# danpovey/quantization

Measured on AMD Instinct MI355X. Metric: vectors encoded/sec at dim=512, 8 codebooks; uint8 codes bit-exact vs ref, higher is better.
Workload: dtype f32 (products: exact 30-bit fixed point on the i8 MFMA); 1 GPU; Quantizer.encode, dim=512, bytes_per_frame=8, codebook_size=256, refine_indexes_iters=5, batch=65536 fp32 Gaussian vectors per GPU (BASELINE.json configs[1]), seeded synthetic codebooks; global_batch=65536, parallelism=batch-sharded x1, no collective

## Files before the change

quantization_amd/csrc/mcq_api.hip:

```cpp
#include "../../include/mcq.h"
#include "../../include/mcq_residual.h"
#include "../../include/mcq_probe.h"
#include "../../include/mcq_wide.h"
#include "../../include/mcq_rerank.h"
#include "mcq_kernels.h"
#include "mcq_fix_kernels.h"
#include "mcq_loss_kernels.h"
#include "mcq_tf_kernels.h"
#include "mcq_pass16_kernels.h"
#include "mcq_train_kernels.h"
#include "mcq_search_kernels.h"
#include "mcq_range_kernels.h"
#include "mcq_wide_kernels.h"
#include "mcq_rerank_kernels.h"

#include <cstdlib>
#include <iterator>
#include <type_traits>
#include <utility>
#include <vector>

using namespace mcq;

namespace {
// ... 179 lines not shown
    void untimed() { open = -1; }
    void end(int category) {
        if (only >= 0 && category != only) { open = -1; return; }
        hipEvent_t e;
        (void)hipEventCreate(&e);
        (void)hipEventRecord(e, stream);
        ev.push_back(e);
        first.push_back(open);
        last.push_back((int)ev.size() - 1);
        cat.push_back(category);
        open = (int)ev.size() - 1;
    }
};

thread_local int g_last_launches = 0;

#define MCQ_LAUNCH_CHECK()                               \
    do {                                                 \
        hipError_t e_ = hipGetLastError();               \
        if (e_ != hipSuccess) return (int)e_;            \
        ++g_last_launches;                               \
    } while (0)

inline int launch_rc() {
    const hipError_t e = hipGetLastError();
    return e == hipSuccess ? 0 : (int)e;
}
inline int counted_launch_rc() { MCQ_LAUNCH_CHECK(); return 0; }

template <typename F>
int launch_in_pieces(long B, int threads_per_row, F &&launch) {
    const long piece = (long)kPieceRows * 64 / (threads_per_row > 64 ? threads_per_row : 64);
    for (long at = 0; at < B; at += piece)
        if (const int rc = launch(at, B - at < piece ? B - at : piece)) return rc;
    return 0;
}

template <int... Vs, typename F>
int pick(int v, F &&f) {
    int rc = MCQ_EUNSUPPORTED;
    (void)((v == Vs && ((rc = f(std::integral_constant<int, Vs>{})), true)) || ...);
    return rc;
}
template <typename F>
int pick_bool(bool b, F &&f) { return b ? f(std::true_type{}) : f(std::false_type{}); }

struct Pair { int a, b; };
template <const auto &Table, typename F, size_t... I>
int pick_pair(int a, int b, F &&f, std::index_sequence<I...>) {
    int rc = MCQ_EUNSUPPORTED;
    (void)((a == Table[I].a && b == Table[I].b &&
            ((rc = f(std::integral_constant<int, Table[I].a>{}, std::integral_constant<int, Table[I].b>{})), true)) || ...);
    return rc;
}
template <const auto &Table, typename F>
int pick_pair(int a, int b, F &&f) { return pick_pair<Table>(a, b, f, std::make_index_sequence<std::size(Table)>{}); }
template <size_t R>
bool in_pairs(const Pair (&table)[R], int a, int b) {
    for (const Pair &p : table) if (p.a == a && p.b == b) return true;
    return false;
}

int allow_dynamic_lds(bool (&allowed)[64], const void *kernel, int bytes) {
    int dev = 0;
    if (hipGetDevice(&dev) != hipSuccess || dev < 0 || dev >= 64) dev = 63;
    if (!allowed[dev] || dev == 63) {
        const hipError_t attr = hipFuncSetAttribute(kernel, hipFuncAttributeMaxDynamicSharedMemorySize, bytes);
        if (attr != hipSuccess) return (int)attr;
        allowed[dev] = true;
    }
    return 0;
}

struct Timed {
    Prof *const prof;
    const int cat;
    Timed(Prof *p, int c) : prof(p), cat(c) { if (prof) prof->begin(cat); }
    ~Timed() { if (prof) prof->end(cat); }
    Timed(const Timed &) = delete;
};

FixRowsArgs fix_rows_args(const float *src, int xh, long R, int D, long ld, int8_t *planes, int *exps, float *xx,
                          const float *bias_src = nullptr, float *bias_dst = nullptr, const float *sub = nullptr,
                          long sub_per = 0, long sub_ld = 0, const float *dot_vec = nullptr, float *dot_out = nullptr) {
    return FixRowsArgs{src, xh, R, fix_round_rows(R), D, ld, fix_round_cols(D), planes, exps, xx, bias_src, bias_dst,
                       sub, sub_per, sub_ld, dot_vec, dot_out, nullptr};
}

int launch_fix_rows(const float *src, int xh, long R, int D, long ld, int8_t *planes, int *exps, float *xx, hipStream_t st,
                    const float *sub = nullptr, unsigned *clear = nullptr) {
    FixRowsArgs a = fix_rows_args(src, xh, R, D, ld, planes, exps, xx, nullptr, nullptr, sub, 0, 0);
    a.clear = clear;
    hipLaunchKernelGGL(k_fix_rows<4>, dim3((unsigned)(a.Rp / 4)), dim3(256), 0, st, a);
    return counted_launch_rc();
}

int launch_fix_rows2(const FixRowsArgs &a, const FixRowsArgs &b, hipStream_t st) {
    const unsigned na = (unsigned)(a.Rp / 4), nb = (unsigned)(b.Rp / 4);
    hipLaunchKernelGGL(k_fix_rows2<4>, dim3(na + nb), dim3(256), 0, st, a, b, na);
    return counted_launch_rc();
}

template <int MODE>
int launch_fgemm(FixGemm g, hipStream_t st) {
    static bool allowed[64] = {};
    constexpr int lds = MODE == FG_SCREEN ? kFixLdsScreen : kFixLds;
    if (const int rc = allow_dynamic_lds(allowed, reinterpret_cast<const void *>(&k_fgemm<MODE>), lds)) return rc;
    const long MT = g.RA / kFixTile, NT = g.RB / kFixTile;
    const int H = (MODE != FG_STORE && g.K > kFixTile) ? g.K / kFixTile : 1;
    const long big = g.walk_rows ? NT : MT, small_units = (g.walk_rows ? MT : NT) / H;
    long units = (big + 7) / 8 * small_units;
    if (units > 32) units = 32;
    hipLaunchKernelGGL((k_fgemm<MODE>), dim3((unsigned)(8 * units)), dim3(512), lds, st, g);
    return counted_launch_rc();
}

int launch_xc(const int8_t *xf, const int *xe, long B, const int8_t *Cf, const int *Ce, long nk, int D, float *out,
              hipStream_t st) {
    FixGemm g{};
    g.A = xf; g.ea = xe; g.RA = fix_round_rows(B); g.M = B;
    g.B = Cf; g.eb = Ce; g.RB = fix_round_rows(nk); g.N = nk;
    g.Dq = fix_round_cols(D);
    g.walk_rows = 0;
    g.out = out; g.ldo = nk;
    return launch_fgemm<FG_STORE>(g, st);
}

inline bool exact_logits_forced() {
    static const bool on = getenv("MCQ_EXACT_LOGITS") && atoi(getenv("MCQ_EXACT_LOGITS")) != 0;
    return on;
}

int launch_logits(const int8_t *xf, const int *xe, long B, const Prepared &P, int N, int K, int D, float lscale,
                  const float *lscale_ptr, float *logits, void *idx, hipStream_t st, unsigned *und_cnt = nullptr,
                  unsigned *und_list = nullptr) {
    const long nk = (long)N * K;
    FixGemm g{};
    g.A = P.Wf; g.ea = P.We; g.RA = fix_round_rows(nk); g.M = nk;
    g.B = xf; g.eb = xe; g.RB = fix_round_rows(B); g.N = B;
    g.Dq = fix_round_cols(D);
    g.walk_rows = 1;
    g.bias = P.bias; g.wmu = P.wmu; g.lscale = lscale; g.lscale_ptr = lscale_ptr;
    g.logits = logits; g.ldo = nk; g.idx = idx; g.idx_wide = K > 256 ? 1 : 0; g.K = K; g.ncb = N;
    if (und_cnt == nullptr) return launch_fgemm<FG_LOGITS>(g, st);
    if (logits != nullptr) return MCQ_EINVAL;
    g.und_cnt = und_cnt; g.und_list = und_list; g.und_cap = (unsigned)(B * N);
    const int rc = launch_fgemm<FG_SCREEN>(g, st);
    if (rc) return rc;
    FixRecheck r{};
    r.W = P.Wf; r.X = xf; r.ew = P.We; r.ex = xe; r.RW = g.RA; r.RX = g.RB; r.Dq = g.Dq;
    r.bias = P.bias; r.wmu = P.wmu; r.lscale_ptr = lscale_ptr; r.lscale = lscale;
    r.idx = idx; r.idx_wide = g.idx_wide; r.K = K; r.ncb = N; r.cnt = und_cnt; r.list = und_list; r.cap = g.und_cap;
    const long waves = B * N;
    hipLaunchKernelGGL(k_fscreen_recheck, dim3((unsigned)(waves < 4096 ? (waves + 3) / 4 : 1024)), dim3(256), 0, st, r);
    return counted_launch_rc();
}

constexpr unsigned kCapStage0 = 32768, kCapWave = 65536;
inline unsigned pass_grid(unsigned full, bool capped, unsigned cap) { return (capped && full > cap) ? cap : full; }

template <typename CT>
int launch_tf_stage0(int K, int N, const float *G, const float *XC, const CT *idx, const float *R, const float *Q, long B, int keep,
                     CT *ent, float *S, CT *fin, const int *nact, const int *map, hipStream_t st, bool capped) {
    const unsigned vgrid = (unsigned)(((B + 3) / 4) * N);
    const dim3 grid(pass_grid(vgrid, capped, kCapStage0)), block(256);
    auto with_k = [&](auto kk) {
        constexpr int KK = kk;
        return pick<1, 2, 4, 8, 16, 32, 64>(N, [&](auto nn) {
            constexpr int NN = nn;
            if constexpr ((KK == 16 && NN >= 4) || KK * NN > kMaxRows) return MCQ_EUNSUPPORTED;
            else return pick_bool(capped, [&](auto strided) {
                constexpr bool STRIDED = strided;
                hipLaunchKernelGGL((k_tf_stage0<KK, NN, STRIDED>), grid, block, 0, st, G, XC, idx, R, Q, B, keep, ent, S, fin, nact, map, vgrid);
                return counted_launch_rc();
            });
        });
    };
    if constexpr (sizeof(CT) == 1) {
        if (K == 16 && N >= 4) {
            const dim3 grid16((unsigned)((B * (N / 4) + 3) / 4));
            return pick<4, 8, 16, 32, 64>(N, [&](auto nn) {
                constexpr int NN = nn;
                hipLaunchKernelGGL((k_tf_stage0_k16<NN>), grid16, block, 0, st, G, XC, idx, R, Q, B, keep, ent, S, nact, map);
                return counted_launch_rc();
            });
        }
        return pick<16, 32, 64, 128, 256>(K, with_k);
    } else {
        return pick<512, 1024>(K, with_k);
    }
}

template <typename CT>
int launch_tf_er(int N, const float *G, const float *XC, const CT *idx, const float *xx, long B, int K, float *E, float *R,
                 float *gterms, long stride, const int *nact, const int *map, hipStream_t st, int form = -1) {
    const dim3 grid((unsigned)((B + 3) / 4)), block(256);
    const bool direct = form < 0 ? B <= 8192 : form == 0;
    return pick<1, 2, 4, 8, 16, 32, 64>(N, [&](auto nn) {
        constexpr int NN = nn, VG = 4 * (64 / NN);
        if constexpr (sizeof(CT) == 2 && NN * 512 > kMaxRows) return MCQ_EUNSUPPORTED;
        else {
            constexpr bool DENSE = sizeof(CT) == 1 && (NN == 4 || NN == 8 || NN == 16);
            if (!direct) {
                const long per = DENSE ? 256 : VG;
                hipLaunchKernelGGL((k_tf_gram_terms<NN, CT, DENSE>), dim3((unsigned)(((B + per - 1) / per) * NN)), block, 0, st, G, idx, B, K,
                                   gterms, nact, stride);
                if (const int rc = counted_launch_rc()) return rc;
                if constexpr (DENSE) {
                    hipLaunchKernelGGL((k_tf_er<NN, CT, true>), dim3((unsigned)((B + VG - 1) / VG)), block, 0, st, gterms, XC, idx, xx, B, K,
                                       E, R, nact, map, static_cast<const float *>(nullptr), stride);
                    return counted_launch_rc();
                }
            }
            hipLaunchKernelGGL((k_tf_er<NN, CT>), grid, block, 0, st, gterms, XC, idx, xx, B, K, E, R, nact, map,
                               direct ? G : static_cast<const float *>(nullptr), stride);
            return counted_launch_rc();
        }
    });
}

constexpr Pair kTfUpLists[] = {{16, 32}, {32, 32}, {32, 64}, {8, 16}, {16, 16}};
constexpr Pair kTfCombLists[] = {{16, 32}, {32, 32}, {32, 64}, {64, 64}, {8, 16}, {16, 16}};

template <typename CT>
constexpr bool tf_comb_reached(int kh, int kc, bool last) {
    const bool wide = sizeof(CT) == 2;
    if (kh == 8 || kc == 16) return !wide && !(kh == kc && last);
    if (kh == 64) return !wide;
    if (kh == kc) return !(last && wide);
    return !(kc == 64 && wide && !last);
}

int launch_tf_up(int kh, int kc, const TfLists &L, long B, int N, int u, int ntab, int per, const float *in, float *out,
                 const int *nact, hipStream_t st) {
    return pick_pair<kTfUpLists>(kh, kc, [&](auto a, auto c) {
        constexpr int KH = a, KC = c;
        hipLaunchKernelGGL((k_tf_up<KH, KC>), dim3((unsigned)(B * ntab)), dim3(64), 0, st, L, B, N, u, ntab, per, in, out, nact);
        return counted_launch_rc();
    });
}

template <typename CT>
int launch_tf_comb(int kh, int kc, const float *E, const TfLists &L, long B, int N, int v, int keep, const float *tabs,
                   CT *fin, const int *nact, hipStream_t st, bool capped) {
    if (fin == nullptr) capped = false;
    const dim3 grid(pass_grid((unsigned)(B * (N >> (v + 1))), capped, kCapWave)), block(64);
    return pick_pair<kTfCombLists>(kh, kc, [&](auto a, auto c) {
        return pick_bool(fin != nullptr, [&](auto last) {
            constexpr int KH = decltype(a)::value, KC = decltype(c)::value;
            constexpr bool LAST = last;
            if constexpr (!tf_comb_reached<CT>(KH, KC, LAST)) return MCQ_EUNSUPPORTED;
            else return pick_bool(capped, [&](auto strided) {
                constexpr bool STRIDED = strided;
                if constexpr (STRIDED && !LAST) return MCQ_EUNSUPPORTED;
                else {
                    hipLaunchKernelGGL((k_tf_comb<KH, KC, LAST, CT, STRIDED>), grid, block, 0, st, E, L, B, N, v, keep, tabs, fin, nact);
                    return counted_launch_rc();
                }
            });
        });
    });
}

enum { CAT_LOGITS = 0, CAT_XX = 1, CAT_STAGE0 = 2, CAT_XC = 3, CAT_LEVEL0 = 4, CAT_LEVEL1 = 5, CAT_TABLES = 6, CAT_COMBINE = 7,
       CAT_TABLES_UP = 8, CAT_COMBINE_UP = 9, CAT_ER = 10, CAT_LEVEL1_FUSED = 11, CAT_TAIL = 12, CAT_COUNT = 13 };
const char *const kCatNames[CAT_COUNT] = {
    "logits_product_argmax",
    "frames_to_limbs",
    "stage0_tables",
    "xc_product",
    "combine_level0",
    "combine_level1",
    "tables_level1",
    "combine_level2",
    "tables_upper_levels",
    "combine_upper_levels",
    "residual_energies",
    "level1_combines_and_tables",
    "encode_tail",
};

template <typename CT, typename F>
int pick_leaf_lists(int K, F &&f) {
    if constexpr (sizeof(CT) == 1) return pick<8, 16>(K == 16 ? 8 : 16, f);
    else return pick<16>(16, f);
}
inline bool pass16_enabled() {
    static const bool on = !(getenv("MCQ_PASS16") && atoi(getenv("MCQ_PASS16")) == 0);
    return on;
}
inline long skip_min_batch() {
    const char *v = getenv("MCQ_SKIP_MIN_BATCH");
    return v ? atol(v) : 8192;
}
constexpr long kErDenseMin = 16384;
inline long er_dense_min() {
    const char *v = getenv("MCQ_ER_DENSE_MIN");
    return v ? atol(v) : kErDenseMin;
}
constexpr long kLazyTablesMin = 16384;
inline long lazy_tables_min() {
    const char *v = getenv("MCQ_LAZY_TABLES_MIN");
    return v ? atol(v) : kLazyTablesMin;
}

template <typename CT>
int run_tf_combines(const float *G, const CT *idx_cur, CT *idx_new, const WorkspaceT<CT> &w, const TfLists &L, long B, int N,
// ... 1737 lines not shown
```

quantization_amd/csrc/mcq_fix_kernels.h:

```cpp
#pragma once
#include "mcq_kernels.h"

namespace mcq {

typedef int i32x4 __attribute__((ext_vector_type(4)));
typedef int i32x16 __attribute__((ext_vector_type(16)));

constexpr int kFixTile = 128;
constexpr int kFixColPad = 128;
constexpr int kFixRing = 4;
constexpr int kFixSlot = 32768;
constexpr int kFixOperand = 16384;
constexpr int kFixInfo = kFixRing * kFixSlot;
constexpr int kFixLds = kFixInfo + 4096;
constexpr int kFixLdsScreen = kFixLds + 1024;

__host__ __device__ inline long fix_round_rows(long r) { return (r + kFixTile - 1) / kFixTile * kFixTile; }
__host__ __device__ inline int fix_round_cols(int d) { return (d + kFixColPad - 1) / kFixColPad * kFixColPad; }
__host__ __device__ inline size_t fix_plane_bytes(long R, int D) { return (size_t)fix_round_rows(R) * fix_round_cols(D) * 4; }

__device__ __forceinline__ int fix_q(float v, int e) {
    float s = ldexpf(v, 30 - e);
    s = fminf(fmaxf(s, -1073741824.0f), 1073741824.0f);
    return (int)rintf(s);
}

struct FixRowsArgs {
    const float *src;
    int xh;
    long R, Rp;
    int D;
    long ld;
    int Dq;
    int8_t *planes;
    int *exps;
    float *xx;
    const float *bias_src;
    float *bias_dst;
    const float *sub;
    long sub_per, sub_ld;
    const float *dot_vec;
    float *dot_out;
    unsigned *clear;
};

template <int RW, bool DOT>
__device__ __forceinline__ void fix_rows_body(const FixRowsArgs &a, unsigned bid) {
    const float *__restrict__ src = a.src;
    const int xh = a.xh, D = a.D, Dq = a.Dq;
    const long R = a.R, Rp = a.Rp, ld = a.ld;
    float *__restrict__ xx = a.xx;
    const float *__restrict__ bias_src = a.bias_src;
    float *__restrict__ bias_dst = a.bias_dst;
    const float *__restrict__ sub = a.sub;
    int8_t *__restrict__ planes = a.planes;
    constexpr int RPW = RW / 4;
    __shared__ __attribute__((aligned(16))) unsigned tile[128 * RW * 4];
    __shared__ int es[RW];
    const int tid = threadIdx.x, lane = tid & 63, wave = tid >> 6;
    const long row0 = (long)bid * RW;
    if (bias_src && tid < RW && row0 + tid < R) bias_dst[row0 + tid] = bias_src[row0 + tid];
    if (a.clear && bid == 0 && tid == 0) *a.clear = 0u;
    const _Float16 *srch = reinterpret_cast<const _Float16 *>(src);
    const bool vec_ok = ((ld & 3) == 0) && ((D & 3) == 0) && ((reinterpret_cast<uintptr_t>(src) & (xh ? 7 : 15)) == 0);
    auto load4 = [&](long row, int q) -> f32x4 {
        f32x4 v = {0.f, 0.f, 0.f, 0.f};
        if (row >= R || 4 * q >= D) return v;
        if (vec_ok) return xh ? load_h4(srch + row * ld + 4 * q) : *reinterpret_cast<const f32x4 *>(src + row * ld + 4 * q);
#pragma unroll
        for (int c = 0; c < 4; ++c)
            if (4 * q + c < D) v[c] = xh ? (float)srch[row * ld + 4 * q + c] : src[row * ld + 4 * q + c];
        return v;
    };
    auto vec4 = [&](const float *p, int q) -> f32x4 {
        f32x4 v = {0.f, 0.f, 0.f, 0.f};
        if (4 * q >= D) return v;
        if (((D & 3) == 0) && ((reinterpret_cast<uintptr_t>(p) & 15) == 0)) return *reinterpret_cast<const f32x4 *>(p + 4 * q);
#pragma unroll
        for (int c = 0; c < 4; ++c)
            if (4 * q + c < D) v[c] = p[4 * q + c];
        return v;
    };
    auto sub4 = [&](long row, int q) -> f32x4 {
        if (!sub || row >= R) return f32x4{0.f, 0.f, 0.f, 0.f};
        return vec4(sub + (a.sub_per ? (row / a.sub_per) * a.sub_ld : 0), q);
    };
    int ev = 0;
    if (DOT && a.dot_vec) {
        float mv = 0.f;
        for (int q = lane; q < (D + 3) / 4; q += 64) {
            const f32x4 v = vec4(a.dot_vec, q);
#pragma unroll
            for (int c = 0; c < 4; ++c) mv = fmaxf(mv, fabsf(v[c]));
        }
        for (int s = 32; s >= 1; s >>= 1) mv = fmaxf(mv, __shfl_xor(mv, s, 64));
        const int be = (int)((__float_as_uint(mv) >> 23) & 0xff);
        ev = (be < 1 ? 1 : be) - 126;
    }
    const bool cached = (RW == 4) && D <= 1024;
    f32x4 cache[RW == 4 ? RPW : 1][4];
#pragma unroll
    for (int rr = 0; rr < RPW; ++rr) {
        const long row = row0 + RPW * wave + rr;
        float m = 0.f, pe = 0.f;
        if (cached) {
            f32x4 raw[4], sv4[4];
#pragma unroll
            for (int j = 0; j < 4; ++j) raw[j] = load4(row, lane + 64 * j);
#pragma unroll
            for (int j = 0; j < 4; ++j) sv4[j] = sub4(row, lane + 64 * j);
#pragma unroll
            for (int j = 0; j < 4; ++j) cache[RW == 4 ? rr : 0][j] = sub ? raw[j] - sv4[j] : raw[j];
#pragma unroll
            for (int j = 0; j < 4; ++j)
#pragma unroll
                for (int c = 0; c < 4; ++c) {
                    m = fmaxf(m, fabsf(cache[RW == 4 ? rr : 0][j][c]));
                    pe = fmaf(cache[RW == 4 ? rr : 0][j][c], cache[RW == 4 ? rr : 0][j][c], pe);
                }
        } else {
            for (int q = lane; q < (D + 3) / 4; q += 64) {
                const f32x4 raw = load4(row, q);
                const f32x4 v = sub ? raw - sub4(row, q) : raw;
#pragma unroll
                for (int c = 0; c < 4; ++c) {
                    m = fmaxf(m, fabsf(v[c]));
                    pe = fmaf(v[c], v[c], pe);
                }
            }
        }
        for (int s = 32; s >= 1; s >>= 1) m = fmaxf(m, __shfl_xor(m, s, 64));
        if (xx) pe = wave_sum_butterfly(pe);
        if (lane == 0) {
            const int be = (int)((__float_as_uint(m) >> 23) & 0xff);
            const int e = (be < 1 ? 1 : be) - 126;
            es[RPW * wave + rr] = e;
            if (row < Rp) a.exps[row] = e;
            if (xx && row < R) xx[row] = pe;
        }
    }
    __syncthreads();
    int T[RPW][4];
#pragma unroll
    for (int rr = 0; rr < RPW; ++rr)
#pragma unroll
        for (int i = 0; i < 4; ++i) T[rr][i] = 0;
    auto limbs4 = [&](const f32x4 &v, int e, unsigned (&w)[4]) {
#pragma unroll
        for (int i = 0; i < 4; ++i) w[i] = 0u;
#pragma unroll
        for (int c = 0; c < 4; ++c) {
            int r = fix_q(v[c], e);
#pragma unroll
            for (int i = 3; i >= 1; --i) {
                const int l = (int)(int8_t)(r & 0xff);
                w[i] |= (unsigned)(l & 0xff) << (8 * c);
                r = (r - l) >> 8;
            }
            w[0] |= (unsigned)(r & 0xff) << (8 * c);
        }
    };
    for (int c0 = 0; c0 < Dq; c0 += 512) {
        const int ncol = (Dq - c0 < 512) ? Dq - c0 : 512;
#pragma unroll
        for (int rr = 0; rr < RPW; ++rr) {
            const int rl = RPW * wave + rr;
            const int e = es[rl];
#pragma unroll
// ... 60 lines not shown
    else fix_rows_body<RW, true>(b, blockIdx.x - blocks_a);
}

enum { FG_STORE = 0, FG_LOGITS = 1, FG_SCREEN = 2 };

struct FixGemm {
    const int8_t *A, *B;
    const int *ea, *eb;
    long RA, RB;
    long M, N;
    int Dq;
    int walk_rows;
    float *out;
    long ldo;
    const float *bias;
    const float *wmu;
    const float *lscale_ptr;
    float lscale;
    float *logits;
    void *idx;
    int idx_wide;
    int K, ncb;
    unsigned *und_cnt, *und_list;
    unsigned und_cap;
};

__device__ __forceinline__ void fg_store_idx(const FixGemm &g, long pos, long entry) {
    if (g.idx_wide) static_cast<uint16_t *>(g.idx)[pos] = (uint16_t)entry;
    else static_cast<uint8_t *>(g.idx)[pos] = (uint8_t)entry;
}

template <int MODE>
__global__ void __launch_bounds__(512)
k_fgemm(const FixGemm g) {
    extern __shared__ __attribute__((aligned(16))) char smem[];
    constexpr bool SCREEN = MODE == FG_SCREEN, LOGITS = MODE != FG_STORE;
    constexpr int NL = SCREEN ? 3 : 4;
    const int tid = threadIdx.x, lane = tid & 63, wave = tid >> 6;
    const int wm = wave & 1, wn = wave >> 1;
    const int r32 = lane & 31, kh = lane >> 5;
    const long MT = g.RA / kFixTile, NT = g.RB / kFixTile;
    const int H = (LOGITS && g.K > kFixTile) ? g.K / kFixTile : 1;
    const long big = g.walk_rows ? NT : MT, small_units = (g.walk_rows ? MT : NT) / H;
    const int xcd = blockIdx.x & 7, slot = blockIdx.x >> 3, per_xcd = gridDim.x >> 3;
    auto tile_of = [&](long t, long &m0, long &n0) -> bool {
        const long unit = t / H, half = t % H;
        const long idx = slot + unit * per_xcd;
        const long bt = (idx / small_units) * 8 + xcd, st = (idx % small_units) * H + half;
        m0 = (g.walk_rows ? st : bt) * kFixTile;
        n0 = (g.walk_rows ? bt : st) * kFixTile;
        return bt < big;
    };
    i32x16 acc[2][NL];
    const int nst = g.Dq / 32;
    const int wu = __builtin_amdgcn_readfirstlane(wave);
    const int op = wu >> 2, chunk = (wu >> 1) & 1, half = wu & 1;
    const long R = op ? g.RB : g.RA;
    const long pl = R * 16, sstride = 8 * R * 16;
    const unsigned dbase = (unsigned)(size_t)smem + op * kFixOperand + (4 * chunk) * 2048 + half * 1024;
    const unsigned voff = lane * 16, voff4 = lane * 4;
    auto base_of = [&](long m0, long n0) { return (op ? g.B + n0 * 16 : g.A + m0 * 16) + (long)(4 * chunk) * R * 16 + half * 1024; };
    auto issue1 = [&](const int8_t *p, int st, int g4) {
        const int8_t *pg = p + g4 * pl;
        const unsigned d = dbase + (st % kFixRing) * kFixSlot + g4 * 2048;
        asm volatile(
            "s_mov_b32 m0, %[d]\n\ts_nop 0\n\t"
            "global_load_lds_dwordx4 %[vo], %[p]\n\t"
            :
            : [vo] "v"(voff), [p] "s"(pg), [d] "s"(d)
            : "memory");
    };
    auto issue_info = [&](long m0, long n0) {
        if (wu < (LOGITS ? 8 : 4)) {
            const void *src = wu < 2 ? static_cast<const void *>(g.ea + m0 + 64 * wu)
                                     : (wu < 4 ? static_cast<const void *>(g.eb + n0 + 64 * (wu - 2))
                                               : (wu < 6 ? static_cast<const void *>(g.bias + m0 + 64 * (wu - 4))
                                                         : static_cast<const void *>(g.wmu + m0 + 64 * (wu - 6))));
            const unsigned d = (unsigned)(size_t)smem + kFixInfo + 256 * (wu < 6 ? wu : wu + 4);
            asm volatile(
                "s_mov_b32 m0, %[d]\n\ts_nop 0\n\t"
                "global_load_lds_dword %[vo], %[p]\n\t"
                :
                : [vo] "v"(voff4), [p] "s"(src), [d] "s"(d)
                : "memory");
        }
    };
    long m0, n0, m0n = 0, n0n = 0;
    if (!tile_of(0, m0, n0)) return;
    const int8_t *pcur = base_of(m0, n0), *pnext = pcur;
    auto step = [&](int st, const i32x4 (&a)[2][NL], const i32x4 (&b)[NL], i32x4 (&an)[2][NL], i32x4 (&bn)[NL]) {
        const char *base = smem + ((st + 1) % kFixRing) * kFixSlot;
        const int8_t *p = (st + 4 < nst) ? pcur + (st + 4) * sstride : pnext + (st + 4 - nst) * sstride;
        constexpr int PI[10] = {0, 0, 1, 0, 1, 2, 0, 1, 2, 3};
        constexpr int PJ[10] = {0, 1, 0, 2, 1, 0, 3, 2, 1, 0};
        constexpr int LO[5] = {0, SCREEN ? 2 : 3, SCREEN ? 4 : 6, SCREEN ? 6 : 8, 10};
#pragma unroll
        for (int g4 = 0; g4 < NL; ++g4) {
            issue1(p, st, g4);
#pragma unroll
            for (int t = 0; t < 2; ++t)
                an[t][g4] = *reinterpret_cast<const i32x4 *>(base + (kh * 4 + g4) * 2048 + (64 * wm + 32 * t + r32) * 16);
            bn[g4] = *reinterpret_cast<const i32x4 *>(base + kFixOperand + (kh * 4 + g4) * 2048 + (32 * wn + r32) * 16);
#pragma unroll
            for (int q = LO[g4]; q < LO[g4 + 1]; ++q)
#pragma unroll
                for (int ta = 0; ta < 2; ++ta)
                    acc[ta][PI[q] + PJ[q]] =
                        __builtin_amdgcn_mfma_i32_32x32x32_i8(a[ta][PI[q]], b[PJ[q]], acc[ta][PI[q] + PJ[q]], 0, 0, 0);
            __builtin_amdgcn_sched_barrier(0);
        }
    };
    i32x4 a0[2][NL], b0[NL], a1[2][NL], b1[NL];
    issue_info(m0, n0);
#pragma unroll
    for (int q = 0; q < 4; ++q)
#pragma unroll
        for (int g4 = 0; g4 < NL; ++g4) issue1(pcur + q * sstride, q, g4);
    if constexpr (SCREEN) asm volatile("s_waitcnt vmcnt(9)" ::: "memory");
    else asm volatile("s_waitcnt vmcnt(12)" ::: "memory");
    __builtin_amdgcn_s_barrier();
#pragma unroll
    for (int l = 0; l < NL; ++l) {
#pragma unroll
        for (int t = 0; t < 2; ++t)
            a0[t][l] = *reinterpret_cast<const i32x4 *>(smem + (kh * 4 + l) * 2048 + (64 * wm + 32 * t + r32) * 16);
        b0[l] = *reinterpret_cast<const i32x4 *>(smem + kFixOperand + (kh * 4 + l) * 2048 + (32 * wn + r32) * 16);
    }
    int *info = reinterpret_cast<int *>(smem + kFixInfo);
    float *infof = reinterpret_cast<float *>(smem + kFixInfo);
    float runv = 0.f;
    int runk = 0;
    float runs = 0.f, runt = 0.f, runq = 0.f;
    int runj = 0, rune = 0;
    for (long t = 0;; ++t) {
        const bool has_next = tile_of(t + 1, m0n, n0n);
        pnext = has_next ? base_of(m0n, n0n) : pcur;
#pragma unroll
        for (int a = 0; a < 2; ++a)
#pragma unroll
            for (int s = 0; s < NL; ++s)
#pragma unroll
                for (int v = 0; v < 16; ++v) acc[a][s][v] = 0;
        for (int st = 0; st < nst; st += 2) {
            if constexpr (SCREEN) asm volatile("s_waitcnt vmcnt(6)\n\ts_waitcnt lgkmcnt(0)" ::: "memory");
            else asm volatile("s_waitcnt vmcnt(8)\n\ts_waitcnt lgkmcnt(0)" ::: "memory");
            __builtin_amdgcn_s_barrier();
            step(st, a0, b0, a1, b1);
            if constexpr (SCREEN) asm volatile("s_waitcnt vmcnt(6)\n\ts_waitcnt lgkmcnt(0)" ::: "memory");
            else asm volatile("s_waitcnt vmcnt(8)\n\ts_waitcnt lgkmcnt(0)" ::: "memory");
            __builtin_amdgcn_s_barrier();
            step(st + 1, a1, b1, a0, b0);
        }
        auto value = [&](int ta, int v, int e) -> float {
            float tt;
            if constexpr (SCREEN) tt = __fmul_rn((float)acc[ta][2][v], 256.0f);
            else tt = __builtin_fmaf((float)acc[ta][2][v], 256.0f, (float)acc[ta][NL - 1][v]);
            tt = __builtin_fmaf((float)acc[ta][1][v], 65536.0f, tt);
            tt = __builtin_fmaf((float)acc[ta][0][v], 16777216.0f, tt);
            return ldexpf(tt, e);
        };
        int rbase = 64 * wm + 4 * kh, cbase = 32 * wn + r32;
        asm volatile("" : "+v"(rbase), "+v"(cbase));
        i32x4 er[2][4];
#pragma unroll
        for (int ta = 0; ta < 2; ++ta)
#pragma unroll
            for (int q = 0; q < 4; ++q) er[ta][q] = *reinterpret_cast<const i32x4 *>(&info[rbase + 32 * ta + 8 * q]);
        const bool full = (m0 + kFixTile <= g.M) && (n0 + kFixTile <= g.N);
        const int ecol = info[128 + cbase] - 36;
        const int rows_left = (int)((g.M - m0 - rbase) > 128 ? 128 : (g.M - m0 - rbase));
        if (MODE == FG_STORE) {
            const bool col_ok = n0 + cbase < g.N;
            float *orow = g.out + (m0 + rbase) * g.ldo + n0 + cbase;
            if (full) {
#pragma unroll
                for (int ta = 0; ta < 2; ++ta)
#pragma unroll
                    for (int v = 0; v < 16; ++v) {
                        const int ro = 32 * ta + 8 * (v >> 2) + (v & 3);
                        orow[(long)ro * g.ldo] = value(ta, v, er[ta][v >> 2][v & 3] + ecol);
                    }
            } else {
#pragma unroll
                for (int ta = 0; ta < 2; ++ta)
#pragma unroll
                    for (int v = 0; v < 16; ++v) {
                        const int ro = 32 * ta + 8 * (v >> 2) + (v & 3);
                        const float val = value(ta, v, er[ta][v >> 2][v & 3] + ecol);
                        if (col_ok && ro < rows_left) orow[(long)ro * g.ldo] = val;
                    }
            }
        } else if constexpr (SCREEN) {
            const float ls = g.lscale_ptr ? *g.lscale_ptr : g.lscale;
            float bv[4], sv[4], tv[4], qm = 0.f;
            int bk[4], sk[4];
            const long col = n0 + cbase;
#pragma unroll
            for (int ta = 0; ta < 2; ++ta) {
#pragma unroll
                for (int v4 = 0; v4 < 4; ++v4) {
                    const f32x4 br4 = *reinterpret_cast<const f32x4 *>(&infof[256 + rbase + 32 * ta + 8 * v4]);
                    const f32x4 wm4 = *reinterpret_cast<const f32x4 *>(&infof[640 + rbase + 32 * ta + 8 * v4]);
#pragma unroll
                    for (int c = 0; c < 4; ++c) {
                        const int v = 4 * v4 + c;
                        const int rl = rbase + 32 * ta + 8 * v4 + c;
                        const float s2 = __fmul_rn(__fadd_rn(value(ta, v, er[ta][v4][c] + ecol), wm4[c]), ls);
                        const float val = __fadd_rn(s2, br4[c]);
                        qm = fmaxf(qm, fmaxf(fabsf(s2), fabsf(val)));
                        const int gi = 2 * ta + (v4 >> 1);
                        if ((v4 & 1) == 0 && c == 0) { bv[gi] = val; bk[gi] = sk[gi] = rl; sv[gi] = tv[gi] = -INFINITY; }
                        else {
                            const bool c1 = val > bv[gi], c2 = val > sv[gi];
                            tv[gi] = __builtin_amdgcn_fmed3f(tv[gi], sv[gi], val);
                            sv[gi] = __builtin_amdgcn_fmed3f(sv[gi], bv[gi], val);
                            sk[gi] = c1 ? bk[gi] : (c2 ? rl : sk[gi]);
                            bk[gi] = c1 ? rl : bk[gi];
                            bv[gi] = fmaxf(bv[gi], val);
                        }
                    }
                }
            }
            int em = info[lane] > info[lane + 64] ? info[lane] : info[lane + 64];
            for (int s = 32; s >= 1; s >>= 1) { const int o = __shfl_xor(em, s, 64); em = o > em ? o : em; }
            auto merge = [](float &b1, int &k1, float &s1, int &j1, float &t1, float b2, int k2, float s2, int j2, float t2) {
                if (b2 > b1) {
                    float f = b1; b1 = b2; b2 = f;
                    f = s1; s1 = s2; s2 = f;
                    t1 = t2;
                    int i = k1; k1 = k2; k2 = i;
                    j1 = j2;
                }
                if (b2 > s1) { t1 = fmaxf(s1, s2); s1 = b2; j1 = k2; }
                else t1 = fmaxf(t1, b2);
            };
            const float cA = 16.5f * 16384.0f * (float)g.Dq;
            auto undecided = [&](float v, float s, float q, int e) {
                const float margin = __fadd_rn(__fadd_rn(__fmul_rn(ldexpf(cA, e + ecol), ls), __fmul_rn(q, 1.9073486328125e-6f)), 7.5231638452626401e-37f);
                return !(__fsub_rn(v, s) > margin);
            };
            auto append = [&](long pos, unsigned second_entry, bool many) {
                const unsigned at = atomicAdd(g.und_cnt, 1u);
                if (at < g.und_cap) {
                    g.und_list[2 * (size_t)at] = (unsigned)pos;
                    g.und_list[2 * (size_t)at + 1] = second_entry | (many ? 0x80000000u : 0u);
                }
            };
            const int K = g.K;
#pragma unroll
            for (int gi = 0; gi < 4; ++gi)
                merge(bv[gi], bk[gi], sv[gi], sk[gi], tv[gi], __shfl_xor(bv[gi], 32, 64), __shfl_xor(bk[gi], 32, 64),
                      __shfl_xor(sv[gi], 32, 64), __shfl_xor(sk[gi], 32, 64), __shfl_xor(tv[gi], 32, 64));
            qm = fmaxf(qm, __shfl_xor(qm, 32, 64));
            if (K >= 32) {
                merge(bv[0], bk[0], sv[0], sk[0], tv[0], bv[1], bk[1], sv[1], sk[1], tv[1]);
                merge(bv[2], bk[2], sv[2], sk[2], tv[2], bv[3], bk[3], sv[3], sk[3], tv[3]);
            }
            if (K >= 64) merge(bv[0], bk[0], sv[0], sk[0], tv[0], bv[2], bk[2], sv[2], sk[2], tv[2]);
            if (K <= 64) {
                if (kh == 0) {
                    const int span = K / 16;
#pragma unroll
                    for (int gi = 0; gi < 4; ++gi) {
                        const long row = m0 + bk[gi];
                        if ((gi % span) == 0 && col < g.N && row < g.M) {
                            fg_store_idx(g, col * g.ncb + row / K, row % K);
                            if (undecided(bv[gi], sv[gi], qm, em))
                                append(col * g.ncb + row / K, (unsigned)((m0 + sk[gi]) % K), undecided(bv[gi], tv[gi], qm, em));
                        }
                    }
                }
            } else {
                float *exv = infof + 384, *exs = infof + 768, *exq = infof + 896;
                int *exk = info + 384 + 128;
                float *ext = reinterpret_cast<float *>(smem + kFixInfo + 4096);
                int *exj = reinterpret_cast<int *>(smem + kFixInfo + 4096 + 512);
                if (wm == 1 && kh == 0) {
                    exv[cbase] = bv[0]; exk[cbase] = bk[0]; exs[cbase] = sv[0]; exq[cbase] = qm;
                    ext[cbase] = tv[0]; exj[cbase] = sk[0];
                }
                asm volatile("s_waitcnt lgkmcnt(0)" ::: "memory");
                __builtin_amdgcn_s_barrier();
                if (wm == 0 && kh == 0) {
                    const int hf = (int)(t % H);
                    float v = bv[0], s = sv[0], t3 = tv[0], q = fmaxf(qm, exq[cbase]);
                    int kk = bk[0], jj = sk[0];
                    merge(v, kk, s, jj, t3, exv[cbase], exk[cbase], exs[cbase], exj[cbase], ext[cbase]);
                    kk += (int)m0;
                    jj += (int)m0;
                    if (hf > 0) {
                        merge(v, kk, s, jj, t3, runv, runk, runs, runj, runt);
                        q = fmaxf(q, runq);
                        em = em > rune ? em : rune;
                    }
                    runv = v; runk = kk; runs = s; runj = jj; runt = t3; runq = q; rune = em;
                    const long k = kk;
                    if (hf == H - 1 && col < g.N && k < g.M) {
                        fg_store_idx(g, col * g.ncb + k / K, k % K);
                        if (undecided(v, s, q, em)) append(col * g.ncb + k / K, (unsigned)(jj % K), undecided(v, t3, q, em));
                    }
                }
            }
        } else {
            const float ls = g.lscale_ptr ? *g.lscale_ptr : g.lscale;
            float bv[4];
            int bk[4];
            const long col = n0 + cbase;
            float *lrow = g.logits ? g.logits + col * g.ldo + m0 + rbase : nullptr;
#pragma unroll
            for (int ta = 0; ta < 2; ++ta) {
#pragma unroll
                for (int v4 = 0; v4 < 4; ++v4) {
                    const f32x4 br4 = *reinterpret_cast<const f32x4 *>(&infof[256 + rbase + 32 * ta + 8 * v4]);
                    const f32x4 wm4 = *reinterpret_cast<const f32x4 *>(&infof[640 + rbase + 32 * ta + 8 * v4]);
                    f32x4 q4;
#pragma unroll
                    for (int c = 0; c < 4; ++c) {
                        const int v = 4 * v4 + c;
                        const int rl = rbase + 32 * ta + 8 * v4 + c;
                        const float val = __fadd_rn(__fmul_rn(__fadd_rn(value(ta, v, er[ta][v4][c] + ecol), wm4[c]), ls), br4[c]);
                        q4[c] = val;
                        const int gi = 2 * ta + (v4 >> 1);
                        if ((v4 & 1) == 0 && c == 0) { bv[gi] = val; bk[gi] = rl; }
                        else if (val > bv[gi]) { bv[gi] = val; bk[gi] = rl; }
                    }
                    if (lrow && (full || (col < g.N && 32 * ta + 8 * v4 < rows_left)))
                        *reinterpret_cast<f32x4 *>(lrow + 32 * ta + 8 * v4) = q4;
                }
            }
            if (g.idx) {
                auto better = [](float v1, int k1, float v2, int k2) { return (v1 > v2) | ((v1 == v2) & (k1 < k2)); };
                const int K = g.K;
#pragma unroll
                for (int gi = 0; gi < 4; ++gi) {
                    const float ov = __shfl_xor(bv[gi], 32, 64);
                    const int ok = __shfl_xor(bk[gi], 32, 64);
                    if (better(ov, ok, bv[gi], bk[gi])) { bv[gi] = ov; bk[gi] = ok; }
                }
                if (K >= 32) {
                    if (bv[1] > bv[0]) { bv[0] = bv[1]; bk[0] = bk[1]; }
                    if (bv[3] > bv[2]) { bv[2] = bv[3]; bk[2] = bk[3]; }
                }
                if (K >= 64 && bv[2] > bv[0]) { bv[0] = bv[2]; bk[0] = bk[2]; }
                if (K <= 64) {
                    if (kh == 0) {
                        const int span = K / 16;
#pragma unroll
                        for (int gi = 0; gi < 4; ++gi) {
                            const long row = m0 + bk[gi];
                            if ((gi % span) == 0 && col < g.N && row < g.M) fg_store_idx(g, col * g.ncb + row / K, row % K);
                        }
                    }
                } else {
                    float *exv = infof + 384;
                    int *exk = info + 384 + 128;
                    if (wm == 1 && kh == 0) { exv[cbase] = bv[0]; exk[cbase] = bk[0]; }
                    asm volatile("s_waitcnt lgkmcnt(0)" ::: "memory");
                    __builtin_amdgcn_s_barrier();
                    if (wm == 0 && kh == 0) {
                        const int hf = (int)(t % H);
                        float v = bv[0];
                        long k = m0 + bk[0];
                        if (better(exv[cbase], exk[cbase], bv[0], bk[0])) { v = exv[cbase]; k = m0 + exk[cbase]; }
                        if (hf > 0 && !(v > runv)) { v = runv; k = runk; }
                        runv = v;
                        runk = (int)k;
                        if (hf == H - 1 && col < g.N && k < g.M) fg_store_idx(g, col * g.ncb + k / K, k % K);
                    }
                }
            }
        }
        if (!has_next) break;
        asm volatile("s_waitcnt lgkmcnt(0)" ::: "memory");
        __builtin_amdgcn_s_barrier();
        m0 = m0n;
        n0 = n0n;
        pcur = pnext;
        issue_info(m0, n0);
    }
    asm volatile("s_waitcnt vmcnt(0)" ::: "memory");
}

struct FixRecheck {
    const int8_t *W, *X;
    const int *ew, *ex;
    long RW, RX;
    int Dq;
    const float *bias, *wmu, *lscale_ptr;
    float lscale;
    void *idx;
    int idx_wide;
    int K, ncb;
    const unsigned *cnt, *list;
    unsigned cap;
};

__global__ void __launch_bounds__(256) k_fscreen_recheck(const FixRecheck a) {
    const int lane = threadIdx.x & 63;
    const unsigned wv = __builtin_amdgcn_readfirstlane(blockIdx.x * 4 + (threadIdx.x >> 6)), nwv = gridDim.x * 4;
    unsigned n = *a.cnt;
    n = n < a.cap ? n : a.cap;
    const float ls = a.lscale_ptr ? *a.lscale_ptr : a.lscale;
    const int K = a.K, nch = a.Dq / 16;
    for (unsigned i = wv; i < n; i += nwv) {
        const unsigned pos = a.list[2 * (size_t)i], snd = a.list[2 * (size_t)i + 1];
        const long col = pos / (unsigned)a.ncb;
        const int cb = (int)(pos % (unsigned)a.ncb);
        const int ecol = a.ex[col] - 36;
        auto chunk = [&](int (&T)[4], int c, long row) {
            i32x4 xl[4], wl[4];
#pragma unroll
            for (int l = 0; l < 4; ++l) {
                xl[l] = *reinterpret_cast<const i32x4 *>(a.X + (((long)c * 4 + l) * a.RX + col) * 16);
                wl[l] = *reinterpret_cast<const i32x4 *>(a.W + (((long)c * 4 + l) * a.RW + row) * 16);
            }
#pragma unroll
            for (int p = 0; p < 4; ++p)
#pragma unroll
                for (int q = 0; p + q < 4; ++q)
#pragma unroll
                    for (int d = 0; d < 4; ++d) T[p + q] = __builtin_amdgcn_sdot4(wl[p][d], xl[q][d], T[p + q], false);
        };
        auto logit = [&](const int (&T)[4], long row) -> float {
            float tt = (float)T[3];
            tt = __builtin_fmaf((float)T[2], 256.0f, tt);
            tt = __builtin_fmaf((float)T[1], 65536.0f, tt);
            tt = __builtin_fmaf((float)T[0], 16777216.0f, tt);
            return __fadd_rn(__fmul_rn(__fadd_rn(ldexpf(tt, a.ew[row] + ecol), a.wmu[row]), ls), a.bias[row]);
        };
        float bv = -INFINITY;
        int bk = 0x7fffffff;
        if ((snd & 0x80000000u) == 0) {
            const int first = a.idx_wide ? (int)static_cast<const uint16_t *>(a.idx)[pos] : (int)static_cast<const uint8_t *>(a.idx)[pos];
            const int j = (lane < 32) ? first : (int)snd;
            const long row = (long)cb * K + j;
            int T[4] = {0, 0, 0, 0};
            for (int c = lane & 31; c < nch; c += 32) chunk(T, c, row);
#pragma unroll
            for (int p = 0; p < 4; ++p)
                for (int sft = 16; sft >= 1; sft >>= 1) T[p] += __shfl_xor(T[p], sft, 64);
            bv = logit(T, row);
            bk = j;
        } else {
            for (int j = lane; j < K; j += 64) {
                const long row = (long)cb * K + j;
                int T[4] = {0, 0, 0, 0};
#pragma unroll 4
                for (int c = 0; c < nch; ++c) chunk(T, c, row);
                const float val = logit(T, row);
                if (j == lane || val > bv) { bv = val; bk = j; }
            }
        }
        for (int s = 32; s >= 1; s >>= 1) {
            const float ov = __shfl_xor(bv, s, 64);
            const int ok = __shfl_xor(bk, s, 64);
            if ((ov > bv) | ((ov == bv) & (ok < bk))) { bv = ov; bk = ok; }
        }
        if (lane == 0) {
            if (a.idx_wide) static_cast<uint16_t *>(a.idx)[pos] = (uint16_t)bk;
            else static_cast<uint8_t *>(a.idx)[pos] = (uint8_t)bk;
        }
    }
}

}
```

Before: 14.52 million vectors/s.

## Pack row index into logit key bits and split recheck into pair and full-scan phases

The screen epilogue now folds bias and wmu*lscale into one precomputed per-row constant in shared memory, so each logit is a single fma. The row id is packed into the low three mantissa bits of the value, which lets the top-3 tracking drop the index bookkeeping. The undecided-margin test is widened to cover that truncation. The recheck kernel moves to 1024-thread blocks: pairwise rechecks run per wave, and full K-scans are spread over the whole block with a shared-memory partial reduction. This trades some extra undecided rows and block-level barriers for a cheaper epilogue and better parallelism on full rescans.

```diff
diff --git a/quantization_amd/csrc/mcq_api.hip b/quantization_amd/csrc/mcq_api.hip
--- a/quantization_amd/csrc/mcq_api.hip
+++ b/quantization_amd/csrc/mcq_api.hip
@@ -355,7 +355,8 @@
     r.bias = P.bias; r.wmu = P.wmu; r.lscale_ptr = lscale_ptr; r.lscale = lscale;
     r.idx = idx; r.idx_wide = g.idx_wide; r.K = K; r.ncb = N; r.cnt = und_cnt; r.list = und_list; r.cap = g.und_cap;
     const long waves = B * N;
-    hipLaunchKernelGGL(k_fscreen_recheck, dim3((unsigned)(waves < 4096 ? (waves + 3) / 4 : 1024)), dim3(256), 0, st, r);
+    constexpr int wpg = kRecheckThreads / 64;
+    hipLaunchKernelGGL(k_fscreen_recheck, dim3((unsigned)(waves < 4096 ? (waves + wpg - 1) / wpg : 4096 / wpg)), dim3(kRecheckThreads), 0, st, r);
     return counted_launch_rc();
 }
 
diff --git a/quantization_amd/csrc/mcq_fix_kernels.h b/quantization_amd/csrc/mcq_fix_kernels.h
--- a/quantization_amd/csrc/mcq_fix_kernels.h
+++ b/quantization_amd/csrc/mcq_fix_kernels.h
@@ -13,7 +13,7 @@
 constexpr int kFixOperand = 16384;
 constexpr int kFixInfo = kFixRing * kFixSlot;
 constexpr int kFixLds = kFixInfo + 4096;
-constexpr int kFixLdsScreen = kFixLds + 1024;
+constexpr int kFixLdsScreen = kFixLds + 1536;
 
 __host__ __device__ inline long fix_round_rows(long r) { return (r + kFixTile - 1) / kFixTile * kFixTile; }
 __host__ __device__ inline int fix_round_cols(int d) { return (d + kFixColPad - 1) / kFixColPad * kFixColPad; }
@@ -380,9 +380,7 @@
             step(st + 1, a1, b1, a0, b0);
         }
         auto value = [&](int ta, int v, int e) -> float {
-            float tt;
-            if constexpr (SCREEN) tt = __fmul_rn((float)acc[ta][2][v], 256.0f);
-            else tt = __builtin_fmaf((float)acc[ta][2][v], 256.0f, (float)acc[ta][NL - 1][v]);
+            float tt = __builtin_fmaf((float)acc[ta][2][v], 256.0f, (float)acc[ta][NL - 1][v]);
             tt = __builtin_fmaf((float)acc[ta][1][v], 65536.0f, tt);
             tt = __builtin_fmaf((float)acc[ta][0][v], 16777216.0f, tt);
             return ldexpf(tt, e);
@@ -420,34 +418,52 @@
             }
         } else if constexpr (SCREEN) {
             const float ls = g.lscale_ptr ? *g.lscale_ptr : g.lscale;
-            float bv[4], sv[4], tv[4], qm = 0.f;
-            int bk[4], sk[4];
             const long col = n0 + cbase;
+            float *crow = reinterpret_cast<float *>(smem + kFixInfo + 4096 + 1024);
+            float qm;
+            {
+                const int rr = 64 * wm + lane;
+                const float b = infof[256 + rr], w = infof[640 + rr];
+                const float c = __builtin_fmaf(w, ls, b);
+                const bool in = m0 + rr < g.M;
+                const bool fin = fabsf(b) < INFINITY && fabsf(w) < INFINITY && fabsf(c) < INFINITY;
+                crow[rr] = in ? c : 0.f;
+                qm = in ? (fin ? fmaxf(fmaxf(fabsf(b), fabsf(w)), fabsf(c)) : INFINITY) : 0.f;
+                for (int s = 32; s >= 1; s >>= 1) qm = fmaxf(qm, __shfl_xor(qm, s, 64));
+            }
+            const float sl = ldexpf(ls, ecol + 8);
+            if (!(sl >= 1.17549435e-38f && sl < INFINITY)) qm = INFINITY;
+            asm volatile("s_waitcnt lgkmcnt(0)" ::: "memory");
+            float bv[4], sv[4], tv[4];
 #pragma unroll
             for (int ta = 0; ta < 2; ++ta) {
 #pragma unroll
                 for (int v4 = 0; v4 < 4; ++v4) {
-                    const f32x4 br4 = *reinterpret_cast<const f32x4 *>(&infof[256 + rbase + 32 * ta + 8 * v4]);
-                    const f32x4 wm4 = *reinterpret_cast<const f32x4 *>(&infof[640 + rbase + 32 * ta + 8 * v4]);
+                    const f32x4 c4 = *reinterpret_cast<const f32x4 *>(&crow[rbase + 32 * ta + 8 * v4]);
 #pragma unroll
                     for (int c = 0; c < 4; ++c) {
                         const int v = 4 * v4 + c;
-                        const int rl = rbase + 32 * ta + 8 * v4 + c;
-                        const float s2 = __fmul_rn(__fadd_rn(value(ta, v, er[ta][v4][c] + ecol), wm4[c]), ls);
-                        const float val = __fadd_rn(s2, br4[c]);
-                        qm = fmaxf(qm, fmaxf(fabsf(s2), fabsf(val)));
+                        float tt = __builtin_fmaf((float)acc[ta][1][v], 256.0f, (float)acc[ta][2][v]);
+                        tt = __builtin_fmaf((float)acc[ta][0][v], 65536.0f, tt);
+                        const float val = __builtin_fmaf(tt, ldexpf(sl, er[ta][v4][c]), c4[c]);
+                        const float key = __uint_as_float((__float_as_uint(val) & ~7u) | (unsigned)(4 * (v4 & 1) + c));
+                        qm = fmaxf(qm, fabsf(key));
                         const int gi = 2 * ta + (v4 >> 1);
-                        if ((v4 & 1) == 0 && c == 0) { bv[gi] = val; bk[gi] = sk[gi] = rl; sv[gi] = tv[gi] = -INFINITY; }
+                        if ((v4 & 1) == 0 && c == 0) { bv[gi] = key; sv[gi] = tv[gi] = -INFINITY; }
                         else {
-                            const bool c1 = val > bv[gi], c2 = val > sv[gi];
-                            tv[gi] = __builtin_amdgcn_fmed3f(tv[gi], sv[gi], val);
-                            sv[gi] = __builtin_amdgcn_fmed3f(sv[gi], bv[gi], val);
-                            sk[gi] = c1 ? bk[gi] : (c2 ? rl : sk[gi]);
-                            bk[gi] = c1 ? rl : bk[gi];
-                            bv[gi] = fmaxf(bv[gi], val);
+                            tv[gi] = __builtin_amdgcn_fmed3f(tv[gi], sv[gi], key);
+                            sv[gi] = __builtin_amdgcn_fmed3f(sv[gi], bv[gi], key);
+                            bv[gi] = __builtin_amdgcn_fmed3f(bv[gi], key, INFINITY);
                         }
                     }
                 }
+            }
+            int bk[4], sk[4];
+#pragma unroll
+            for (int gi = 0; gi < 4; ++gi) {
+                const unsigned ib = __float_as_uint(bv[gi]) & 7u, is = __float_as_uint(sv[gi]) & 7u;
+                bk[gi] = rbase + 16 * gi + (int)(2 * (ib & 4u) + (ib & 3u));
+                sk[gi] = rbase + 16 * gi + (int)(2 * (is & 4u) + (is & 3u));
             }
             int em = info[lane] > info[lane + 64] ? info[lane] : info[lane + 64];
             for (int s = 32; s >= 1; s >>= 1) { const int o = __shfl_xor(em, s, 64); em = o > em ? o : em; }
@@ -463,9 +479,11 @@
                 else t1 = fmaxf(t1, b2);
             };
             const float cA = 16.5f * 16384.0f * (float)g.Dq;
+            const float cU = ldexpf(__builtin_fmaf(ls, 2.168404344971009e-19f, 1.0f), -78);
             auto undecided = [&](float v, float s, float q, int e) {
-                const float margin = __fadd_rn(__fadd_rn(__fmul_rn(ldexpf(cA, e + ecol), ls), __fmul_rn(q, 1.9073486328125e-6f)), 7.5231638452626401e-37f);
-                return !(__fsub_rn(v, s) > margin);
+                const float y1 = ldexpf(cA, e + ecol);
+                const float margin = __fadd_rn(__fadd_rn(__fmul_rn(y1, ls), __fmul_rn(q, 3.814697265625e-6f)), cU);
+                return !(y1 < 1.2676506002282294e30f) | !(margin < 1.2676506002282294e30f) | !(__fsub_rn(v, s) > margin);
             };
             auto append = [&](long pos, unsigned second_entry, bool many) {
                 const unsigned at = atomicAdd(g.und_cnt, 1u);
@@ -609,6 +627,7 @@
     asm volatile("s_waitcnt vmcnt(0)" ::: "memory");
 }
 
+constexpr int kRecheckThreads = 1024;
 struct FixRecheck {
     const int8_t *W, *X;
     const int *ew, *ex;
@@ -623,71 +642,111 @@
     unsigned cap;
 };
 
-__global__ void __launch_bounds__(256) k_fscreen_recheck(const FixRecheck a) {
-    const int lane = threadIdx.x & 63;
-    const unsigned wv = __builtin_amdgcn_readfirstlane(blockIdx.x * 4 + (threadIdx.x >> 6)), nwv = gridDim.x * 4;
+__global__ void __launch_bounds__(kRecheckThreads) k_fscreen_recheck(const FixRecheck a) {
+    __shared__ int part[kRecheckThreads * 4];
+    __shared__ float wbv[kRecheckThreads / 64];
+    __shared__ int wbk[kRecheckThreads / 64];
+    const int tid = threadIdx.x, lane = tid & 63, wave = tid >> 6;
+    const unsigned wv = __builtin_amdgcn_readfirstlane(blockIdx.x * (kRecheckThreads / 64) + wave), nwv = gridDim.x * (kRecheckThreads / 64);
     unsigned n = *a.cnt;
     n = n < a.cap ? n : a.cap;
     const float ls = a.lscale_ptr ? *a.lscale_ptr : a.lscale;
     const int K = a.K, nch = a.Dq / 16;
+    auto chunk = [&](int (&T)[4], int c, long row, long col) {
+        i32x4 xl[4], wl[4];
+#pragma unroll
+        for (int l = 0; l < 4; ++l) {
+            xl[l] = *reinterpret_cast<const i32x4 *>(a.X + (((long)c * 4 + l) * a.RX + col) * 16);
+            wl[l] = *reinterpret_cast<const i32x4 *>(a.W + (((long)c * 4 + l) * a.RW + row) * 16);
+        }
+#pragma unroll
+        for (int p = 0; p < 4; ++p)
+#pragma unroll
+            for (int q = 0; p + q < 4; ++q)
+#pragma unroll
+                for (int d = 0; d < 4; ++d) T[p + q] = __builtin_amdgcn_sdot4(wl[p][d], xl[q][d], T[p + q], false);
+    };
+    auto logit = [&](const int (&T)[4], long row, int ecol) -> float {
+        float tt = (float)T[3];
+        tt = __builtin_fmaf((float)T[2], 256.0f, tt);
+        tt = __builtin_fmaf((float)T[1], 65536.0f, tt);
+        tt = __builtin_fmaf((float)T[0], 16777216.0f, tt);
+        return __fadd_rn(__fmul_rn(__fadd_rn(ldexpf(tt, a.ew[row] + ecol), a.wmu[row]), ls), a.bias[row]);
+    };
+    auto better = [](float v1, int k1, float v2, int k2) { return (v1 > v2) | ((v1 == v2) & (k1 < k2)); };
+    auto store = [&](unsigned pos, int k) {
+        if (a.idx_wide) static_cast<uint16_t *>(a.idx)[pos] = (uint16_t)k;
+        else static_cast<uint8_t *>(a.idx)[pos] = (uint8_t)k;
+    };
     for (unsigned i = wv; i < n; i += nwv) {
         const unsigned pos = a.list[2 * (size_t)i], snd = a.list[2 * (size_t)i + 1];
+        if (snd & 0x80000000u) continue;
+        const long col = pos / (unsigned)a.ncb;
+        const int cb = (int)(pos % (unsigned)a.ncb);
+        const int first = a.idx_wide ? (int)static_cast<const uint16_t *>(a.idx)[pos] : (int)static_cast<const uint8_t *>(a.idx)[pos];
+        const int j = (lane < 32) ? first : (int)snd;
+        const long row = (long)cb * K + j;
+        int T[4] = {0, 0, 0, 0};
+        for (int c = lane & 31; c < nch; c += 32) chunk(T, c, row, col);
+#pragma unroll
+        for (int p = 0; p < 4; ++p)
+            for (int sft = 16; sft >= 1; sft >>= 1) T[p] += __shfl_xor(T[p], sft, 64);
+        const float bv = logit(T, row, a.ex[col] - 36);
+        const float ov = __shfl_xor(bv, 32, 64);
+        const int ok = __shfl_xor(j, 32, 64);
+        if (lane == 0) store(pos, better(ov, ok, bv, j) ? ok : j);
+    }
+    const int P = K < kRecheckThreads ? kRecheckThreads / K : 1;
+    for (unsigned i = blockIdx.x; i < n; i += gridDim.x) {
+        const unsigned pos = a.list[2 * (size_t)i], snd = a.list[2 * (size_t)i + 1];
+        if ((snd & 0x80000000u) == 0) continue;
         const long col = pos / (unsigned)a.ncb;
         const int cb = (int)(pos % (unsigned)a.ncb);
         const int ecol = a.ex[col] - 36;
-        auto chunk = [&](int (&T)[4], int c, long row) {
-            i32x4 xl[4], wl[4];
-#pragma unroll
-            for (int l = 0; l < 4; ++l) {
-                xl[l] = *reinterpret_cast<const i32x4 *>(a.X + (((long)c * 4 + l) * a.RX + col) * 16);
-                wl[l] = *reinterpret_cast<const i32x4 *>(a.W + (((long)c * 4 + l) * a.RW + row) * 16);
-            }
-#pragma unroll
-            for (int p = 0; p < 4; ++p)
-#pragma unroll
-                for (int q = 0; p + q < 4; ++q)
-#pragma unroll
-                    for (int d = 0; d < 4; ++d) T[p + q] = __builtin_amdgcn_sdot4(wl[p][d], xl[q][d], T[p + q], false);
-        };
-        auto logit = [&](const int (&T)[4], long row) -> float {
-            float tt = (float)T[3];
-            tt = __builtin_fmaf((float)T[2], 256.0f, tt);
-            tt = __builtin_fmaf((float)T[1], 65536.0f, tt);
-            tt = __builtin_fmaf((float)T[0], 16777216.0f, tt);
-            return __fadd_rn(__fmul_rn(__fadd_rn(ldexpf(tt, a.ew[row] + ecol), a.wmu[row]), ls), a.bias[row]);
-        };
         float bv = -INFINITY;
         int bk = 0x7fffffff;
-        if ((snd & 0x80000000u) == 0) {
-            const int first = a.idx_wide ? (int)static_cast<const uint16_t *>(a.idx)[pos] : (int)static_cast<const uint8_t *>(a.idx)[pos];
-            const int j = (lane < 32) ? first : (int)snd;
+        if (P > 1) {
+            const int j = tid % K, p = tid / K;
             const long row = (long)cb * K + j;
             int T[4] = {0, 0, 0, 0};
-            for (int c = lane & 31; c < nch; c += 32) chunk(T, c, row);
-#pragma unroll
-            for (int p = 0; p < 4; ++p)
-                for (int sft = 16; sft >= 1; sft >>= 1) T[p] += __shfl_xor(T[p], sft, 64);
-            bv = logit(T, row);
-            bk = j;
+            if (p < P)
+                for (int c = p; c < nch; c += P) chunk(T, c, row, col);
+#pragma unroll
+            for (int s = 0; s < 4; ++s) part[tid * 4 + s] = T[s];
+            __syncthreads();
+            if (tid < K) {
+                for (int pp = 1; pp < P; ++pp)
+#pragma unroll
+                    for (int s = 0; s < 4; ++s) T[s] += part[(pp * K + tid) * 4 + s];
+                const float val = logit(T, row, ecol);
+                bv = val != val ? -INFINITY : val;
+                bk = j;
+            }
         } else {
-            for (int j = lane; j < K; j += 64) {
+            for (int j = tid; j < K; j += kRecheckThreads) {
                 const long row = (long)cb * K + j;
                 int T[4] = {0, 0, 0, 0};
 #pragma unroll 4
-                for (int c = 0; c < nch; ++c) chunk(T, c, row);
-                const float val = logit(T, row);
-                if (j == lane || val > bv) { bv = val; bk = j; }
+                for (int c = 0; c < nch; ++c) chunk(T, c, row, col);
+                float val = logit(T, row, ecol);
+                val = val != val ? -INFINITY : val;
+                if (j == tid || val > bv) { bv = val; bk = j; }
             }
         }
         for (int s = 32; s >= 1; s >>= 1) {
             const float ov = __shfl_xor(bv, s, 64);
             const int ok = __shfl_xor(bk, s, 64);
-            if ((ov > bv) | ((ov == bv) & (ok < bk))) { bv = ov; bk = ok; }
-        }
-        if (lane == 0) {
-            if (a.idx_wide) static_cast<uint16_t *>(a.idx)[pos] = (uint16_t)bk;
-            else static_cast<uint8_t *>(a.idx)[pos] = (uint8_t)bk;
-        }
+            if (better(ov, ok, bv, bk)) { bv = ov; bk = ok; }
+        }
+        if (lane == 0) { wbv[wave] = bv; wbk[wave] = bk; }
+        __syncthreads();
+        if (tid == 0) {
+#pragma unroll
+            for (int w = 1; w < kRecheckThreads / 64; ++w)
+                if (better(wbv[w], wbk[w], bv, bk)) { bv = wbv[w]; bk = wbk[w]; }
+            store(pos, bk);
+        }
+        __syncthreads();
     }
 }
 
```

Result: no change. 14.47 million vectors/s (-0.4%).
